# luzbetak/rag-faiss-embedding

Measured on NVIDIA B200. Metric: queries/sec @k=10 (flat L2, 384-d), higher is better.
Workload: dtype bf16 tensor-core candidates + f32 exact re-rank

## Files before the change

### rag-faiss-embedding_b200/csrc/gemm_topk_sm100.cu

```cuda
#include <cuda.h>
#include <math.h>
#include <stdlib.h>

#include "common.cuh"
#include "rerank.cuh"

namespace b2f {

namespace k2 {

constexpr int BM = 128;
constexpr int BN = 256;
constexpr int BK = 64;
constexpr int UMMA_K = 16;
constexpr int STAGES_HEAP = 3;
constexpr int STAGES_LIST = 4;
constexpr int STAGES_QRES = 3;
constexpr int QRES_MAX_KB = 6;
constexpr int LIST_CAP_MIN = 128;
constexpr int JSLOTS = 16;
constexpr int A_BYTES = BM * BK * 2;
constexpr int B_BYTES = BN * BK * 2;
constexpr int STAGE_BYTES = A_BYTES + B_BYTES;
constexpr int EPI_THREADS = 128;
// ... 759 lines not shown
#pragma unroll
                    for (int c4 = 0; c4 < 8; c4++)
                        *reinterpret_cast<uint4*>(st + ((c4 ^ (lane & 7)) << 2)) = make_uint4(r[4 * c4], r[4 * c4 + 1], r[4 * c4 + 2], r[4 * c4 + 3]);
                    uint32_t m = mask;
                    while (m) {
                        const int j = __ffs(m) - 1;
                        m &= m - 1;
                        const float sdot = __uint_as_float(st[((((j >> 2) ^ (lane & 7)) << 2)) + (j & 3)]);
                        const float key = L2 ? fmaf(-2.f, sdot, tbc[j]) : tbc[j] - sdot;
                        if (cnt < la.cap) mylist[cnt] = make_uint2(__float_as_uint(key), (uint32_t)(rowc + j));
                        cnt++;
                        if (jv == 1) {
                            best[JSLOTS - 1] = fminf(best[JSLOTS - 1], key);
                        } else if (key < best[JSLOTS - 1]) {
                            float nb[JSLOTS];
#pragma unroll
                            for (int i = 0; i < JSLOTS; i++) nb[i] = fmaxf(i > 0 ? best[i - 1] : -kInf, fminf(best[i], key));
#pragma unroll
                            for (int i = 0; i < JSLOTS; i++) best[i] = nb[i];
                        }
                    }
                }
            };
            const int seg_tiles = seg_tiles_of(sgi);
#pragma unroll 1
            for (int t = 0; t < seg_tiles; t++, gt++) {
                const int acc = gt & 1;
                const uint32_t acc_phase = (gt >> 1) & 1;
                if (la.early && active && t >= 2 && (t < 8 || (t < 32 && (t & 3) == 0) || (t & la.period_mask) == 0)) refresh(true);
                const uint32_t rmask = t == 0 ? 0xffffffffu : (t == 1 ? 0x55555555u
                                     : ((!la.early && (t < 8 || (t < 32 && (t & 3) == 0) || (t & 15) == 0)) ? 1u : 0u));
                mbar_wait(&bias_full[acc], acc_phase);
                mbar_wait(&tmem_full[acc], acc_phase);
                tc_fence_after();
                const int32_t row0 = tile_row0[acc] + half * COLS;
                const float* tb = bias + acc * BN + half * COLS;
                const uint32_t tile_taddr = lane_taddr + (uint32_t)(acc * BN + half * COLS);
                uint32_t ra[32], rb[32];
                tmem_ld32(tile_taddr, ra);
#pragma unroll 1
                for (int c = 0; c < COLS / 32; c += 2) {
                    tmem_ld_wait();
                    tmem_ld32(tile_taddr + (uint32_t)((c + 1) * 32), rb);
                    process(ra, ((rmask >> c) & 1u) != 0u, false, tb + c * 32, row0 + c * 32);
                    tmem_ld_wait();
                    if (c + 2 < COLS / 32) tmem_ld32(tile_taddr + (uint32_t)((c + 2) * 32), ra);
                    process(rb, ((rmask >> (c + 1)) & 1u) != 0u, t == 0 && c == 0, tb + (c + 1) * 32, row0 + (c + 1) * 32);
                }
                tc_fence_before();
                __syncwarp();
                if (lane == 0) {
                    if constexpr (PAIR) {
                        mbar_arrive(&bias_empty[acc]);
                        mbar_arrive_cluster(&tmem_empty[acc], 0);
                    } else {
                        mbar_arrive(&tmem_empty[acc]);
                    }
                }
            }
            if (warp == 4 && lane == 0) K2_STAMP(4);
            if (active) {
                const int have = cnt <= la.cap ? cnt : 0;
                refresh(true);
                int w = 0;
#pragma unroll 1
                for (int i0 = 0; i0 < have; i0 += 16) {
                    uint2 e[16];
#pragma unroll
                    for (int u = 0; u < 16; u++) e[u] = (i0 + u < have) ? mylist[i0 + u] : make_uint2(0x7f800000u, 0u);
#pragma unroll
                    for (int u = 0; u < 16; u++)
                        if (i0 + u < have && __uint_as_float(e[u].x) <= thr) mylist[w++] = e[u];
                }
                la.counts[(int64_t)qrow * la.nl_stride + vsplit] = cnt > la.cap ? cnt : w;
                la.final_thr[(int64_t)qrow * la.nl_stride + vsplit] = thr;
            }
            if (warp == 4 && lane == 0) K2_STAMP(5);
            }
        } else {
            const int qrow = seg[0].qtile * BM + tid;
            const bool active = qrow < nq;
            for (int j = 0; j < KP; j++) {
                heap_k[j * EPI_THREADS + tid] = FLT_MAX;
                heap_i[j * EPI_THREADS + tid] = -1;
            }
            float thr = FLT_MAX;
            const int heap_tiles = seg_tiles_of(0);
            for (int t = 0; t < heap_tiles; t++) {
                const int acc = t & 1;
                const uint32_t acc_phase = (t >> 1) & 1;
                mbar_wait(&bias_full[acc], acc_phase);
                mbar_wait(&tmem_full[acc], acc_phase);
                tc_fence_after();
                const int32_t row0 = tile_row0[acc];
                const float* tb = bias + acc * BN;
                const uint32_t tile_taddr = lane_taddr + (uint32_t)(acc * BN);
#pragma unroll 1
                for (int c = 0; c < BN / 32; c++) {
                    uint32_t r[32];
                    tmem_ld32(tile_taddr + (uint32_t)(c * 32), r);
                    tmem_ld_wait();
                    const float* tbc = tb + c * 32;
                    const uint32_t mask = active ? chunk_mask(r, tbc, thr) : 0u;
                    uint32_t um = __reduce_or_sync(kFull, mask);
                    while (um) {
                        const int j = __ffs(um) - 1;
                        um &= um - 1;
                        const uint32_t v = pick(r, j);
                        if (mask & (1u << j)) {
                            const float sdot = __uint_as_float(v);
                            const float key = L2 ? fmaf(-2.f, sdot, tbc[j]) : tbc[j] - sdot;
                            if (key < thr) thr = heap_push<KP>(heap_k, heap_i, tid, key, row0 + c * 32 + j);
                        }
                    }
                }
                tc_fence_before();
                __syncwarp();
                if (lane == 0) mbar_arrive(&tmem_empty[acc]);
            }
            if (active) {
                for (int m = KP - 1; m > 0; m--) {
                    const float lk_ = heap_k[m * EPI_THREADS + tid];
                    const int32_t li_ = heap_i[m * EPI_THREADS + tid];
                    heap_k[m * EPI_THREADS + tid] = heap_k[tid];
                    heap_i[m * EPI_THREADS + tid] = heap_i[tid];
                    heap_sift_down_n<KP>(heap_k, heap_i, tid, m, lk_, li_);
                }
                float* ok = pk + ((int64_t)qrow * nsplits + split) * KP;
                int32_t* oi = pi + ((int64_t)qrow * nsplits + split) * KP;
                for (int j = 0; j < KP; j++) {
                    ok[j] = heap_k[j * EPI_THREADS + tid];
                    oi[j] = heap_i[j * EPI_THREADS + tid];
                }
            }
        }
    }
    tc_fence_before();
    __syncthreads();
    if constexpr (PAIR) cluster_sync_all();
    if (threadIdx.x == 0) K2_STAMP(6);
    if (warp == 2) {
        tc_fence_after();
        if constexpr (PAIR)
            asm volatile("tcgen05.dealloc.cta_group::2.sync.aligned.b32 %0, %1;" ::"r"(tmem_base), "r"((uint32_t)TMEM_COLS) : "memory");
        else
            asm volatile("tcgen05.dealloc.cta_group::1.sync.aligned.b32 %0, %1;" ::"r"(tmem_base), "r"((uint32_t)TMEM_COLS) : "memory");
        if (lane == 0) K2_STAMP(7);
    }
}

constexpr int MERGE_THREADS = kRerankThreads;
constexpr int MERGE_MAX = 4096;
constexpr int RANK_MAX = 1024;
constexpr int KP_MAX = 256;
static_assert(MERGE_MAX == kRangeHitsMax, "range search stages as many entries per query as the merge holds");

__device__ __forceinline__ int block_count_le(const unsigned long long* comp, int M, unsigned long long bound, int* s_cnt,
                                              int it, int tid, int lane) {
    if (tid == 0) s_cnt[(it + 1) % 3] = 0;
    int c = 0;
    for (int i = tid; i < M; i += MERGE_THREADS) c += comp[i] <= bound ? 1 : 0;
    c = __reduce_add_sync(kFull, c);
    if (lane == 0 && c) atomicAdd(&s_cnt[it % 3], c);
    __syncthreads();
    return s_cnt[it % 3];
}

__device__ __forceinline__ void radix_pick(int* s_hist, int* s_wsum, int* s_sel, int shift, unsigned int& lo, int& need,
                                           int tid, int lane, int warp) {
    __syncthreads();
    const int h = s_hist[tid];
    int incl = h;
#pragma unroll
    for (int d = 1; d < 32; d <<= 1) {
        const int up = __shfl_up_sync(kFull, incl, d);
        if (lane >= d) incl += up;
    }
    if (lane == 31) s_wsum[warp] = incl;
    __syncthreads();
    int base = 0;
    for (int w = 0; w < warp; w++) base += s_wsum[w];
    incl += base;
    if (incl >= need && incl - h < need) {
        s_sel[0] = tid;
        s_sel[1] = need - (incl - h);
    }
    __syncthreads();
    lo |= (unsigned int)s_sel[0] << shift;
    need = s_sel[1];
    __syncthreads();
}

__global__ void __launch_bounds__(MERGE_THREADS)
merge_lists_kernel(const uint2* __restrict__ cand, const int32_t* __restrict__ counts, const float* __restrict__ final_thr,
                   int nl_stride, int tile_queries, int ntile_units, int total_units, int halves, int kp, int list_cap,
                   int cap_entries, unsigned long long* __restrict__ total_entries, const uint8_t* __restrict__ only_flagged,
                   const RerankArgs ra) {
    extern __shared__ __align__(16) unsigned long long comp[];
    if (only_flagged && !only_flagged[blockIdx.x]) return;
    __shared__ int s_off[2 * kNumSMs + 2];
    __shared__ int s_cnt[3];
    __shared__ int s_nsurv, s_nrest;
    __shared__ int s_hist[MERGE_THREADS], s_wsum[MERGE_THREADS / 32], s_sel[2];
    __shared__ int s_ovf;
    __shared__ unsigned int s_tc_enc;
    const int cap_c = cap_entries > RANK_MAX ? cap_entries : RANK_MAX;
    unsigned long long* surv = comp + cap_c;
    float* sk = reinterpret_cast<float*>(surv + KP_MAX);
    int32_t* si = reinterpret_cast<int32_t*>(sk + RANK_MAX);
    unsigned short* owner = reinterpret_cast<unsigned short*>(si + RANK_MAX);
    float* ek = reinterpret_cast<float*>(comp);
    int32_t* ei = reinterpret_cast<int32_t*>(ek + RANK_MAX);
    const int q = blockIdx.x, tid = threadIdx.x, lane = tid & 31, warp = tid >> 5;
    const int tile = q / tile_queries;
    int nsplits;
    {
        const TileInfo ti = tile_info(tile, ntile_units, total_units, 0, halves);
        nsplits = (ti.nfw + ti.nsw) * halves;
    }
    if (tid == 0) {
        s_tc_enc = 0xffffffffu;
        s_ovf = 0;
        s_nsurv = 0;
        s_nrest = 0;
        s_cnt[0] = 0;
    }
    __syncthreads();
    {
        float tc = 3.0e38f;
        int o = 0;
        for (int s2 = tid; s2 < nsplits; s2 += MERGE_THREADS) {
            int c = counts[(int64_t)q * nl_stride + s2];
            tc = fminf(tc, final_thr[(int64_t)q * nl_stride + s2]);
            if (c > list_cap) {
                c = list_cap;
                o = 1;
            }
            s_off[s2 + 1] = c;
        }
#pragma unroll
        for (int d = 16; d >= 1; d >>= 1) tc = fminf(tc, __shfl_xor_sync(kFull, tc, d));
        o = __reduce_or_sync(kFull, o);
        if (lane == 0) {
            atomicMin(&s_tc_enc, enc_key(tc));
            if (o) s_ovf = 1;
        }
    }
    __syncthreads();
    if (warp == 0) {
        int run = 0;
        for (int s0 = 0; s0 < nsplits; s0 += 32) {
            const int s2 = s0 + lane;
            const int c = s2 < nsplits ? s_off[s2 + 1] : 0;
            int incl = c;
#pragma unroll
            for (int d = 1; d < 32; d <<= 1) {
                const int up = __shfl_up_sync(kFull, incl, d);
                if (lane >= d) incl += up;
            }
            __syncwarp();
            if (s2 < nsplits) s_off[s2 + 1] = run + incl;
            run += __shfl_sync(kFull, incl, 31);
        }
        if (lane == 0) {
            s_off[0] = 0;
            if (total_entries) atomicAdd(total_entries, (unsigned long long)run);
            if (run > cap_entries && (ra.range || !ra.certify)) s_ovf = 1;
        }
    }
    __syncthreads();
    if (ra.out_map && ra.out_map[q] < 0) return;
    if (s_ovf) {
        if (tid == 0) rerank_record_failure(ra, q, true);
        return;
    }
    int M = s_off[nsplits];
    const bool big = M > cap_entries;
    if (big) {
        unsigned int lo = 0;
        int need = kp;
#pragma unroll 1
        for (int pass = 0; pass < 4; pass++) {
            const int shift = 24 - 8 * pass;
            s_hist[tid] = 0;
            __syncthreads();
#pragma unroll 1
            for (int l = 0; l < nsplits; l++) {
                const int c = s_off[l + 1] - s_off[l];
                const uint2* p = cand + ((int64_t)q * nl_stride + l) * list_cap;
                for (int j0 = 0; j0 < c; j0 += MERGE_THREADS) {
                    const int j = j0 + tid;
                    const unsigned int key = j < c ? enc_key(__uint_as_float(p[j].x)) : 0u;
                    const bool in = j < c && (pass == 0 || (key >> (shift + 8)) == (lo >> (shift + 8)));
                    const unsigned int bin = (key >> shift) & 255u;
                    const unsigned int peers = __match_any_sync(kFull, in ? bin : 256u + (unsigned)lane);
                    if (in && lane == __ffs(peers) - 1) atomicAdd(&s_hist[bin], __popc(peers));
                }
            }
            radix_pick(s_hist, s_wsum, s_sel, shift, lo, need, tid, lane, warp);
        }
#pragma unroll 1
        for (int l = 0; l < nsplits; l++) {
            const int c = s_off[l + 1] - s_off[l];
            const uint2* p = cand + ((int64_t)q * nl_stride + l) * list_cap;
            for (int j = tid; j < c; j += MERGE_THREADS) {
                const uint2 e = p[j];
                const unsigned int key = enc_key(__uint_as_float(e.x));
                if (key <= lo) {
                    const int slot = atomicAdd(&s_nrest, 1);
                    if (slot < cap_entries) comp[slot] = ((unsigned long long)key << 32) | (unsigned long long)e.y;
                }
            }
        }
        __syncthreads();
        M = s_nrest;
        __syncthreads();
        if (tid == 0) s_nrest = 0;
        if (M > cap_entries) {
            if (tid == 0) rerank_record_failure(ra, q, true);
            return;
        }
        __syncthreads();
    } else {
    for (int l = tid; l < nsplits; l += MERGE_THREADS) {
        const int o = s_off[l], e = s_off[l + 1];
        for (int i = o; i < e; i++) owner[i] = (unsigned short)l;
    }
    __syncthreads();
    for (int i0 = tid; i0 < M; i0 += 4 * MERGE_THREADS) {
        uint2 e[4];
#pragma unroll
        for (int u = 0; u < 4; u++) {
            const int i = i0 + u * MERGE_THREADS;
            e[u] = make_uint2(0u, 0u);
            if (i < M) {
                const int l = owner[i];
                e[u] = cand[((int64_t)q * nl_stride + l) * list_cap + (i - s_off[l])];
            }
        }
#pragma unroll
        for (int u = 0; u < 4; u++) {
            const int i = i0 + u * MERGE_THREADS;
            if (i < M) comp[i] = ((unsigned long long)enc_key(__uint_as_float(e[u].x)) << 32) | (unsigned long long)e[u].y;
        }
    }
    }
    __syncthreads();
    if (M <= MERGE_THREADS) {
        if (tid < M) {
            const unsigned long long mine = comp[tid];
            int rank = 0;
            for (int j = 0; j < M; j++) rank += comp[j] < mine ? 1 : 0;
            sk[rank] = dec_key((uint32_t)(mine >> 32));
            si[rank] = (int32_t)(uint32_t)(mine & 0xffffffffu);
        }
    } else {
        unsigned long long T = ~0ull;
        int it = 0;
        unsigned int lo = 0;
        int need = kp;
#pragma unroll 1
        for (int pass = 0; pass < 4; pass++) {
            const int shift = 24 - 8 * pass;
            s_hist[tid] = 0;
            __syncthreads();
            for (int i0 = 0; i0 < M; i0 += MERGE_THREADS) {
                const int i = i0 + tid;
                const unsigned int key = i < M ? (unsigned int)(comp[i] >> 32) : 0u;
                const bool in = i < M && (pass == 0 || (key >> (shift + 8)) == (lo >> (shift + 8)));
                const unsigned int bin = (key >> shift) & 255u;
                const unsigned int peers = __match_any_sync(kFull, in ? bin : 256u + (unsigned)lane);
                if (in && lane == __ffs(peers) - 1) atomicAdd(&s_hist[bin], __popc(peers));
            }
            radix_pick(s_hist, s_wsum, s_sel, shift, lo, need, tid, lane, warp);
        }
        const unsigned long long kbits = (unsigned long long)lo << 32;
        T = kbits | 0xffffffffull;
        if (block_count_le(comp, M, T, s_cnt, it++, tid, lane) > kp) {
            unsigned int ilo = 0, ihi = 0xffffffffu;
            while (ilo < ihi) {
                const unsigned int mid = ilo + ((ihi - ilo) >> 1);
                const int total = block_count_le(comp, M, kbits | mid, s_cnt, it++, tid, lane);
                if (total >= kp) ihi = mid;
                else ilo = mid + 1;
            }
            T = kbits | ilo;
        }
        for (int i = tid; i < M; i += MERGE_THREADS) {
            const unsigned long long v = comp[i];
            if (v <= T) {
                const int slot = atomicAdd(&s_nsurv, 1);
                if (slot < kp) surv[slot] = v;
            } else if (M <= RANK_MAX) {
                const int slot = kp + atomicAdd(&s_nrest, 1);
                if (slot < RANK_MAX) {
                    sk[slot] = dec_key((uint32_t)(v >> 32));
                    si[slot] = (int32_t)(uint32_t)(v & 0xffffffffu);
                }
            }
        }
        __syncthreads();
        const int ns = s_nsurv < kp ? s_nsurv : kp;
        for (int t = tid; t < ns; t += MERGE_THREADS) {
            const unsigned long long mine = surv[t];
            int rank = 0;
            for (int j = 0; j < ns; j++) rank += surv[j] < mine ? 1 : 0;
            sk[rank] = dec_key((uint32_t)(mine >> 32));
            si[rank] = (int32_t)(uint32_t)(mine & 0xffffffffu);
        }
    }
    __syncthreads();
    const float tc = dec_key(s_tc_enc);
    const int nc1 = M < kp ? M : kp;
    const float bound1 = (M > kp || big) ? fminf(sk[kp - 1], tc) : tc;
    __shared__ float s_tau_last;
    bool cert = false;
    if (ra.range) {
        if (M <= RANK_MAX) cert = rerank_block(ra, q, sk, si, M, tc, false, ek, ei, &s_tau_last);
        else if (tid == 0) s_tau_last = FLT_MAX;
    } else {
        if (ra.certify && ra.stage1 >= ra.k && ra.stage1 < nc1)
            cert = rerank_block(ra, q, sk, si, ra.stage1, fminf(sk[ra.stage1], tc), false, ek, ei, &s_tau_last);
        if (!cert) cert = rerank_block(ra, q, sk, si, nc1, bound1, M < kp, ek, ei, &s_tau_last);
        if (!cert && ra.certify && !big && M > kp && M <= RANK_MAX) {
            cert = rerank_block(ra, q, sk, si, M, tc, false, ek, ei, &s_tau_last);
            if (tid == 0 && cert) atomicAdd(ra.fail_count + 4, 1);
        }
    }
    if (tid == 0 && ra.certify && !cert) rerank_record_failure(ra, q, false, s_tau_last);
}

constexpr int WM_WARPS = 8;
constexpr int WM_MAX = 128;
constexpr int WM_LISTS = 64;

__device__ __forceinline__ bool warp_rerank(const RerankArgs& a, int q, const float* sk, const int32_t* si, int nc, float bound,
                                            bool all_rows, float* ek, int32_t* ei, int lane, float& tau_out) {
    const float* qv = a.q + (int64_t)q * a.d;
    const bool l2 = a.metric == B2F_METRIC_L2;
    const int sl = lane & 7;
    for (int c0 = 0; c0 < nc; c0 += 4) {
        const int c = c0 + (lane >> 3);
        int32_t id = c < nc ? si[c] : -1;
        if ((int64_t)id >= a.ntotal) id = -1;
        const float key = exact_key_8lanes(a, qv, id, sl, l2);
        if (sl == 0 && c < nc) {
            const bool ok = id >= 0 && !(key != key);
            ek[c] = ok ? key : FLT_MAX;
            ei[c] = ok ? id : -1;
        }
    }
    __syncwarp();
    float tau = FLT_MAX;
    for (int t = lane; t < nc; t += 32) {
        const float mk = ek[t];
        const int32_t mi = ei[t];
        int rank = 0;
        for (int j = 0; j < nc; j++) {
            const float ok_ = ek[j];
            const int32_t oi_ = ei[j];
            rank += (cand_less(ok_, oi_, mk, mi) || (ok_ == mk && oi_ == mi && j < t)) ? 1 : 0;
        }
        if (rank < a.k) {
            const int64_t o = (int64_t)q * a.k + rank;
            a.D[o] = mi < 0 ? (l2 ? FLT_MAX : -FLT_MAX) : (l2 ? mk : -mk);
            a.I[o] = mi < 0 ? -1 : (int64_t)mi + a.id_offset;
        }
        if (rank == a.k - 1) tau = mk;
    }
    for (int t = nc + lane; t < a.k; t += 32) {
        a.D[(int64_t)q * a.k + t] = l2 ? FLT_MAX : -FLT_MAX;
        a.I[(int64_t)q * a.k + t] = -1;
    }
#pragma unroll
    for (int d = 16; d >= 1; d >>= 1) tau = fminf(tau, __shfl_xor_sync(kFull, tau, d));
    __syncwarp();
    tau_out = tau;
    return all_rows || rerank_certified(a, q, tau, bound);
}

__global__ void __launch_bounds__(WM_WARPS * 32)
merge_lists_warp_kernel(const uint2* __restrict__ cand, const int32_t* __restrict__ counts, const float* __restrict__ final_thr,
                        int nl_stride, int tile_queries, int ntile_units, int total_units, int halves, int kp, int list_cap,
                        unsigned long long* __restrict__ total_entries, uint8_t* __restrict__ big_flag, int nq, const RerankArgs ra) {
    __shared__ __align__(16) unsigned long long s_comp[WM_WARPS][WM_MAX];
    __shared__ float s_sk[WM_WARPS][WM_MAX], s_ek[WM_WARPS][WM_MAX];
    __shared__ int32_t s_si[WM_WARPS][WM_MAX], s_ei[WM_WARPS][WM_MAX];
    const int warp = threadIdx.x >> 5, lane = threadIdx.x & 31;
    const int q = blockIdx.x * WM_WARPS + warp;
    if (q >= nq) return;
    unsigned long long* comp = s_comp[warp];
    float* sk = s_sk[warp];
    int32_t* si = s_si[warp];
    int nlists;
    {
        const TileInfo ti = tile_info(q / tile_queries, ntile_units, total_units, 0, halves);
        nlists = (ti.nfw + ti.nsw) * halves;
    }
    int c0 = 0, c1 = 0;
    float tc = 3.0e38f;
    bool ovf = false;
    if (lane < nlists) {
        c0 = counts[(int64_t)q * nl_stride + lane];
        tc = fminf(tc, final_thr[(int64_t)q * nl_stride + lane]);
    }
    if (lane + 32 < nlists) {
        c1 = counts[(int64_t)q * nl_stride + lane + 32];
        tc = fminf(tc, final_thr[(int64_t)q * nl_stride + lane + 32]);
    }
    ovf = c0 > list_cap || c1 > list_cap;
    int i0 = c0, i1 = c1;
#pragma unroll
    for (int d = 1; d < 32; d <<= 1) {
        const int u0 = __shfl_up_sync(kFull, i0, d), u1 = __shfl_up_sync(kFull, i1, d);
        if (lane >= d) { i0 += u0; i1 += u1; }
    }
    const int tot0 = __shfl_sync(kFull, i0, 31), M = tot0 + __shfl_sync(kFull, i1, 31);
#pragma unroll
    for (int d = 16; d >= 1; d >>= 1) tc = fminf(tc, __shfl_xor_sync(kFull, tc, d));
    ovf = __any_sync(kFull, ovf);
    if (lane == 0 && total_entries) atomicAdd(total_entries, (unsigned long long)(ovf ? 0 : M));
    if (ovf || M > WM_MAX) {
        if (lane == 0) big_flag[q] = 1;
        return;
    }
    if (lane == 0) big_flag[q] = 0;
    {
        const uint2* l0 = cand + ((int64_t)q * nl_stride + lane) * list_cap;
        const int o0 = i0 - c0;
        for (int i = 0; i < c0; i++) {
            const uint2 e = l0[i];
            comp[o0 + i] = ((unsigned long long)enc_key(__uint_as_float(e.x)) << 32) | (unsigned long long)e.y;
        }
        const uint2* l1 = cand + ((int64_t)q * nl_stride + lane + 32) * list_cap;
        const int o1 = tot0 + i1 - c1;
        for (int i = 0; i < c1; i++) {
            const uint2 e = l1[i];
            comp[o1 + i] = ((unsigned long long)enc_key(__uint_as_float(e.x)) << 32) | (unsigned long long)e.y;
        }
    }
    __syncwarp();
    for (int t = lane; t < M; t += 32) {
        const unsigned long long mine = comp[t];
        int rank = 0;
        for (int j = 0; j < M; j++) rank += comp[j] < mine ? 1 : 0;
        sk[rank] = dec_key((uint32_t)(mine >> 32));
        si[rank] = (int32_t)(uint32_t)(mine & 0xffffffffu);
    }
    __syncwarp();
    const int nc1 = M < kp ? M : kp;
    const float bound1 = (M > kp) ? fminf(sk[kp - 1], tc) : tc;
    bool cert = false;
    float tau = FLT_MAX;
    if (ra.certify && ra.stage1 >= ra.k && ra.stage1 < nc1)
        cert = warp_rerank(ra, q, sk, si, ra.stage1, fminf(sk[ra.stage1], tc), false, s_ek[warp], s_ei[warp], lane, tau);
    if (!cert) cert = warp_rerank(ra, q, sk, si, nc1, bound1, M < kp, s_ek[warp], s_ei[warp], lane, tau);
    if (!cert && ra.certify && M > kp) {
        cert = warp_rerank(ra, q, sk, si, M, tc, false, s_ek[warp], s_ei[warp], lane, tau);
        if (lane == 0 && cert) atomicAdd(ra.fail_count + 4, 1);
    }
    if (lane == 0 && ra.certify && !cert) rerank_record_failure(ra, q, false, tau);
}

typedef CUresult (*EncodeTiledFn)(CUtensorMap*, CUtensorMapDataType, cuuint32_t, void*, const cuuint64_t*, const cuuint64_t*,
                                  const cuuint32_t*, const cuuint32_t*, CUtensorMapInterleave, CUtensorMapSwizzle,
                                  CUtensorMapL2promotion, CUtensorMapFloatOOBfill);

static EncodeTiledFn get_encode() {
    static EncodeTiledFn fn = nullptr;
    if (!fn) {
        void* p = nullptr;
        cudaDriverEntryPointQueryResult qres;
        if (cudaGetDriverEntryPoint("cuTensorMapEncodeTiled", &p, cudaEnableDefault, &qres) == cudaSuccess &&
            qres == cudaDriverEntryPointSuccess)
            fn = reinterpret_cast<EncodeTiledFn>(p);
    }
    return fn;
}
// ... 244 lines not shown
    plan->units = units;
    plan->nsplits = units / plan->tile_units;
    if (!plan->list_mode) {
        plan->nlists = plan->nsplits;
        plan->list_j = kp;
        plan->list_g = 1;
        plan->list_cap = 0;
        return B2F_OK;
    }
    plan->nlists = nseg_max * halves;
    const int j = nv_min;
    plan->list_j = j;
    plan->list_g = (kp + j - 1) / j;
    {
        int r = 2 * ((units + plan->tile_units - 1) / plan->tile_units);
        if (r < 2) r = 2;
        if (r > 512) r = 512;
        const char* e = getenv("B200FLAT_ROUND_TILES");
        if (e && atoi(e) >= 1 && atoi(e) <= 4096) r = atoi(e);
        plan->round_tiles = r;
    }
    {
        const double rows_per_list = (double)n * plan->tile_units / units / halves;
        const double expected = 32.0 + (j + 2.5) * log(rows_per_list > 64.0 ? rows_per_list / 32.0 : 2.0);
        int cap = (int)(2.5 * expected);
        cap = (cap + 63) / 64 * 64;
        if (cap < k2::LIST_CAP_MIN) cap = k2::LIST_CAP_MIN;
        if (cap > 1024) cap = 1024;
        plan->list_cap = cap;
    }
    return B2F_OK;
}

int plan_unit_work(int T, int U, int R, int64_t ntiles, int kp, int unit, int32_t* seg_info, int64_t* tiles, int64_t cap, int32_t* counts) {
    if (T < 1 || U < T || R < 1 || ntiles < 0 || kp < 1 || unit < 0 || unit >= U || !seg_info || !counts) return -1;
    k2::Seg seg[2];
    const int nseg = k2::unit_segments(unit, T, U, kp, k2::EPI_WARPS_LIST / 4, seg);
    for (int s = 0; s < nseg; s++) {
        seg_info[7 * s + 0] = seg[s].qtile;
        seg_info[7 * s + 1] = seg[s].slot;
        seg_info[7 * s + 2] = seg[s].nv;
        seg_info[7 * s + 3] = (int32_t)seg[s].p0;
        seg_info[7 * s + 4] = (int32_t)seg[s].p1;
        seg_info[7 * s + 5] = seg[s].j;
        seg_info[7 * s + 6] = seg[s].g;
        k2::SegIter it;
        it.init(seg[s].p0, seg[s].p1, U, R, ntiles);
        int32_t c = 0;
        for (int64_t t; (t = it.next()) >= 0; c++)
            if (tiles && c < cap) tiles[(int64_t)s * cap + c] = t;
        counts[s] = c;
    }
    return nseg;
}

int launch_tensor_scan(const __nv_bfloat16* scan, int64_t dpad, const float* norms, int64_t n, int metric,
                       const __nv_bfloat16* qb, int nq, int nq_pad, const TensorScanPlan& plan, float* pk, int32_t* pi,
                       const TensorScanLists& lists, cudaStream_t st) {
    struct MapKey {
        const void* base;
        uint64_t inner, rows;
        uint32_t box;
        bool operator==(const MapKey& o) const { return base == o.base && inner == o.inner && rows == o.rows && box == o.box; }
    };
    static thread_local MapKey kq{}, kx{};
    static thread_local CUtensorMap mq, mx;
    const MapKey nkq{qb, (uint64_t)dpad, (uint64_t)nq_pad, (uint32_t)k2::BM};
    const MapKey nkx{scan, (uint64_t)dpad, (uint64_t)n, (uint32_t)(plan.pair_mode ? k2::BN / 2 : k2::BN)};
    if (!(nkq == kq)) {
        B2F_TRY(k2::make_map(&mq, qb, (uint64_t)dpad, (uint64_t)nq_pad, (uint64_t)dpad, k2::BM));
        kq = nkq;
    }
    if (!(nkx == kx)) {
        B2F_TRY(k2::make_map(&mx, scan, (uint64_t)dpad, (uint64_t)n, (uint64_t)dpad, nkx.box));
        kx = nkx;
    }
    const int kblocks = (int)(dpad / k2::BK);
    const bool l2 = metric == B2F_METRIC_L2;
    k2::ListArgs la{};
    if (plan.list_mode) {
        la.shared_thr = lists.shared_thr;
        la.cand = reinterpret_cast<uint2*>(lists.cand);
        la.counts = lists.counts;
        la.kp = plan.kp;
        la.nl_stride = plan.nlists;
        la.cap = plan.list_cap;
        la.final_thr = lists.final_thr;
        {
            static int early = -1;
            if (early < 0) {
                const char* e = getenv("B200FLAT_EARLY_REFRESH");
                early = (e && e[0] == '0') ? 0 : 1;
            }
            la.early = early;
            static int period = -1;
            if (period < 0) {
                const char* e = getenv("B200FLAT_REFRESH_PERIOD");
                period = e ? atoi(e) : 32;
                if (period != 2 && period != 4 && period != 8 && period != 16 && period != 32 && period != 64 && period != 128) period = 32;
            }
            la.period_mask = period - 1;
            static int keep = -1;
            if (keep < 0) {
                const char* e = getenv("B200FLAT_L2_KEEP");
                keep = (e && e[0] == '1') ? 1 : 0;
            }
            la.l2_keep = keep;
            static int die_mode = -1;
            if (die_mode < 0) {
                const char* e = getenv("B200FLAT_DIE_MODE");
                die_mode = e ? atoi(e) : 1;
                if (die_mode < 0 || die_mode > 3) die_mode = 1;
            }
            la.die_mode = (lists.die_ctr && plan.tile_units > 1) ? die_mode : 0;
            la.die_ctr = lists.die_ctr;
            la.bal_T = plan.tile_units;
            la.bal_U = plan.units;
            la.bal_R = plan.round_tiles;
            la.range_thr = lists.range_thr;
        }
        if (plan.pair_mode)
            return l2 ? k2::launch_k2<0, true, true, true, true>(mq, mx, norms, n, nq, kblocks, plan, pk, pi, la, st)
                      : k2::launch_k2<0, false, true, true, true>(mq, mx, norms, n, nq, kblocks, plan, pk, pi, la, st);
        if (kblocks <= k2::QRES_MAX_KB)
            return l2 ? k2::launch_k2<0, true, true, true>(mq, mx, norms, n, nq, kblocks, plan, pk, pi, la, st)
                      : k2::launch_k2<0, false, true, true>(mq, mx, norms, n, nq, kblocks, plan, pk, pi, la, st);
        return l2 ? k2::launch_k2<0, true, true, false>(mq, mx, norms, n, nq, kblocks, plan, pk, pi, la, st)
                  : k2::launch_k2<0, false, true, false>(mq, mx, norms, n, nq, kblocks, plan, pk, pi, la, st);
    }
    if (plan.kp == 32)
        return l2 ? k2::launch_k2<32, true, false, false>(mq, mx, norms, n, nq, kblocks, plan, pk, pi, la, st)
                  : k2::launch_k2<32, false, false, false>(mq, mx, norms, n, nq, kblocks, plan, pk, pi, la, st);
    if (plan.kp == 64)
        return l2 ? k2::launch_k2<64, true, false, false>(mq, mx, norms, n, nq, kblocks, plan, pk, pi, la, st)
                  : k2::launch_k2<64, false, false, false>(mq, mx, norms, n, nq, kblocks, plan, pk, pi, la, st);
    set_error("tensor scan: k' = %d not supported", plan.kp);
    return B2F_EINVAL;
}

int launch_merge_lists(const TensorScanLists& lists, int nq, const TensorScanPlan& plan, unsigned long long* total_entries,
                       const RerankArgs& ra, cudaStream_t st) {
    if (nq <= 0) return B2F_OK;
    if (plan.kp > k2::KP_MAX || plan.nlists > 2 * kNumSMs) {
        set_error("merge: k' = %d / %d lists per query not supported", plan.kp, plan.nlists);
        return B2F_EINVAL;
    }
    int cap_entries = plan.nlists * plan.list_cap;
    const int expect = 4 * (plan.kp + 3 * plan.nlists);
    if (cap_entries > expect) cap_entries = expect;
    if (cap_entries < k2::RANK_MAX) cap_entries = k2::RANK_MAX;
    if (cap_entries > k2::MERGE_MAX) cap_entries = k2::MERGE_MAX;
    const int cap_c = cap_entries > k2::RANK_MAX ? cap_entries : k2::RANK_MAX;
    const size_t smem = (size_t)cap_c * 8 + (size_t)k2::KP_MAX * 8 + (size_t)k2::RANK_MAX * 8 + (size_t)cap_entries * 2;
    {
        static bool configured[kMaxDevices] = {};
        const int dev = current_device_slot();
        std::lock_guard<std::mutex> lk(launch_cache_mutex());
        if (!configured[dev]) {
            B2F_CUDA(cudaFuncSetAttribute(k2::merge_lists_kernel, cudaFuncAttributeMaxDynamicSharedMemorySize,
                                          (int)((size_t)k2::MERGE_MAX * 10 + (size_t)k2::KP_MAX * 8 + (size_t)k2::RANK_MAX * 8)));
            configured[dev] = true;
        }
    }
    const uint8_t* only_flagged = nullptr;
    static int warp_env = -1;
    if (warp_env < 0) {
        const char* e = getenv("B200FLAT_WARP_MERGE");
        warp_env = e ? atoi(e) : 8192;
    }
    if (warp_env > 0 && nq >= warp_env && lists.big_flag && plan.nlists <= k2::WM_LISTS && plan.kp <= k2::WM_MAX / 2 && ra.D &&
        !ra.range && !ra.out_map) {
        k2::merge_lists_warp_kernel<<<(nq + k2::WM_WARPS - 1) / k2::WM_WARPS, k2::WM_WARPS * 32, 0, st>>>(
            reinterpret_cast<const uint2*>(lists.cand), lists.counts, lists.final_thr, plan.nlists, plan.pair_mode ? 2 * k2::BM : k2::BM,
            plan.tile_units, plan.units, k2::EPI_WARPS_LIST / 4, plan.kp, plan.list_cap, total_entries, lists.big_flag, nq, ra);
        B2F_CUDA(cudaGetLastError());
        only_flagged = lists.big_flag;
        total_entries = nullptr;
    }
    k2::merge_lists_kernel<<<nq, k2::MERGE_THREADS, smem, st>>>(reinterpret_cast<const uint2*>(lists.cand), lists.counts, lists.final_thr,
                                                               plan.nlists, plan.pair_mode ? 2 * k2::BM : k2::BM, plan.tile_units, plan.units,
                                                               k2::EPI_WARPS_LIST / 4, plan.kp, plan.list_cap, cap_entries, total_entries,
                                                               only_flagged, ra);
    B2F_CUDA(cudaGetLastError());
    return B2F_OK;
}

int launch_range_collect(const TensorScanLists& lists, int nq, const TensorScanPlan& plan, float tau, const RerankArgs& ra,
                         float* skey, int32_t* sid, int32_t* staged, int32_t* count, int32_t* scan_list, int32_t* scan_n,
                         cudaStream_t st) {
    if (nq <= 0) return B2F_OK;
    if (!plan.list_mode || plan.nlists > 2 * kNumSMs) {
        set_error("range collect: a LIST-mode plan of at most %d lists per query is required", 2 * kNumSMs);
        return B2F_EINVAL;
    }
    k2::range_collect_kernel<<<nq, k2::MERGE_THREADS, 0, st>>>(reinterpret_cast<const uint2*>(lists.cand), lists.counts, lists.range_thr,
                                                               plan.nlists, plan.pair_mode ? 2 * k2::BM : k2::BM, plan.tile_units,
                                                               plan.units, k2::EPI_WARPS_LIST / 4, plan.list_cap, tau, ra, skey, sid,
                                                               staged, count, scan_list, scan_n);
    B2F_CUDA(cudaGetLastError());
    return B2F_OK;
}

}

#ifdef B2F_K2_TRACE
extern "C" __attribute__((visibility("default"))) int b2f_debug_k2_trace(unsigned long long* out, int n) {
    if (n > 2 * b2f::kNumSMs * 12) n = 2 * b2f::kNumSMs * 12;
    if (cudaMemcpyFromSymbol(out, b2f::k2::g_k2_trace, (size_t)n * 8) != cudaSuccess) return -1;
    static unsigned long long zeros[2 * b2f::kNumSMs * 12] = {};
    return cudaMemcpyToSymbol(b2f::k2::g_k2_trace, zeros, sizeof(zeros)) == cudaSuccess ? 0 : -1;
}
#endif
```

### rag-faiss-embedding_b200/csrc/rerank.cuh

```cuda
#pragma once
#include "common.cuh"

namespace b2f {

constexpr int kRerankThreads = 256;

__device__ __forceinline__ float exact_key_8lanes(const RerankArgs& a, const float* __restrict__ qv, int32_t id, int sl, bool l2) {
    float acc = 0.f;
    if (id >= 0) {
        if (a.rows_f32 && (a.d & 3) == 0) {
            const float* x = a.rows_f32 + (int64_t)id * a.d;
            for (int j0 = sl * 4; j0 < a.d; j0 += 128) {
                float4 xv[4], qq[4];
#pragma unroll
                for (int u = 0; u < 4; u++) {
                    const int j = j0 + 32 * u;
                    xv[u] = j < a.d ? __ldg(reinterpret_cast<const float4*>(x + j)) : make_float4(0.f, 0.f, 0.f, 0.f);
                }
#pragma unroll
                for (int u = 0; u < 4; u++) {
                    const int j = j0 + 32 * u;
                    qq[u] = j < a.d ? __ldg(reinterpret_cast<const float4*>(qv + j)) : make_float4(0.f, 0.f, 0.f, 0.f);
                }
#pragma unroll
                for (int u = 0; u < 4; u++) {
                    if (l2) {
                        const float t0 = xv[u].x - qq[u].x, t1 = xv[u].y - qq[u].y, t2 = xv[u].z - qq[u].z, t3 = xv[u].w - qq[u].w;
                        acc = fmaf(t0, t0, acc); acc = fmaf(t1, t1, acc); acc = fmaf(t2, t2, acc); acc = fmaf(t3, t3, acc);
                    } else {
                        acc = fmaf(xv[u].x, qq[u].x, acc); acc = fmaf(xv[u].y, qq[u].y, acc);
                        acc = fmaf(xv[u].z, qq[u].z, acc); acc = fmaf(xv[u].w, qq[u].w, acc);
                    }
                }
            }
        } else if (!a.rows_f32 && (a.d & 7) == 0) {
            const __nv_bfloat16* x = a.rows_bf16 + (int64_t)id * a.pitch_bf16;
            for (int j0 = sl * 8; j0 < a.d; j0 += 128) {
                uint4 w[2];
#pragma unroll
                for (int u = 0; u < 2; u++) {
                    const int j = j0 + 64 * u;
                    w[u] = j < a.d ? __ldg(reinterpret_cast<const uint4*>(x + j)) : make_uint4(0u, 0u, 0u, 0u);
                }
#pragma unroll
                for (int u = 0; u < 2; u++) {
                    const int j = j0 + 64 * u;
                    if (j < a.d) {
                        const uint32_t ww[4] = {w[u].x, w[u].y, w[u].z, w[u].w};
                        const float4 qa = __ldg(reinterpret_cast<const float4*>(qv + j));
                        const float4 qb = __ldg(reinterpret_cast<const float4*>(qv + j + 4));
                        const float qq[8] = {qa.x, qa.y, qa.z, qa.w, qb.x, qb.y, qb.z, qb.w};
                        float mm[8] = {0.f, 0.f, 0.f, 0.f, 0.f, 0.f, 0.f, 0.f};
                        if (a.centre) {
                            const float4 ma = __ldg(reinterpret_cast<const float4*>(a.centre + j));
                            const float4 mb = __ldg(reinterpret_cast<const float4*>(a.centre + j + 4));
                            mm[0] = ma.x; mm[1] = ma.y; mm[2] = ma.z; mm[3] = ma.w; mm[4] = mb.x; mm[5] = mb.y; mm[6] = mb.z; mm[7] = mb.w;
                        }
#pragma unroll
                        for (int h = 0; h < 4; h++) {
                            const float x0 = mm[2 * h] + __uint_as_float(ww[h] << 16), x1 = mm[2 * h + 1] + __uint_as_float(ww[h] & 0xffff0000u);
                            if (l2) {
                                const float t0 = x0 - qq[2 * h], t1 = x1 - qq[2 * h + 1];
                                acc = fmaf(t0, t0, acc); acc = fmaf(t1, t1, acc);
                            } else {
                                acc = fmaf(x0, qq[2 * h], acc); acc = fmaf(x1, qq[2 * h + 1], acc);
                            }
                        }
                    }
                }
            }
        } else {
            for (int j = sl; j < a.d; j += 8) {
                const float xv = a.rows_f32 ? a.rows_f32[(int64_t)id * a.d + j]
                                            : (a.centre ? a.centre[j] : 0.f) + __bfloat162float(a.rows_bf16[(int64_t)id * a.pitch_bf16 + j]);
                if (l2) {
                    const float t = xv - qv[j];
                    acc = fmaf(t, t, acc);
                } else {
                    acc = fmaf(xv, qv[j], acc);
                }
            }
        }
    }
    acc += __shfl_xor_sync(kFull, acc, 4);
    acc += __shfl_xor_sync(kFull, acc, 2);
    acc += __shfl_xor_sync(kFull, acc, 1);
    return l2 ? acc : -acc;
}

__device__ __forceinline__ bool rerank_certified(const RerankArgs& a, int q, float tau, float bound) {
    const bool l2 = a.metric == B2F_METRIC_L2;
    const float qn2 = a.qnorm[q];
    const float qn = sqrtf(qn2);
    const float eq = a.qerr[q];
    const float gam = 4.f * (float)(a.d + 16) * 5.9604645e-8f;
    if (l2) {
        const float nu = gam * (2.f * qn * a.max_row_norm + qn2 + a.max_row_norm * a.max_row_norm);
        const float c = bound + qn2 - nu;
        const float L = sqrtf(fmaxf(c, 0.f)) - eq - a.max_row_err;
        return L > 0.f && L * L * (1.f - 4e-7f) > tau;
    }
    const float cq = a.qconst ? a.qconst[q] : 0.f;
    const float xmax = a.max_row_norm + a.max_row_err + a.mu_norm;
    const float nu = gam * qn * a.max_row_norm + 2.4e-7f * (a.mu_norm * (xmax + qn + eq + a.mu_norm) + qn * a.max_row_norm);
    const float U = -bound + cq + nu + (qn + eq) * a.max_row_err + a.max_row_norm * eq;
    return U < -tau;
}

__device__ __forceinline__ bool rerank_block(const RerankArgs& a, int q, const float* ck, const int32_t* ci, int nc, float bound,
                                             bool all_rows, float* ek, int32_t* ei, float* tau_out = nullptr) {
    __shared__ float s_tau;
    __shared__ int s_cert;
    const int lane = threadIdx.x & 31;
    const float* qv = a.q + (int64_t)q * a.d;
    const bool l2 = a.metric == B2F_METRIC_L2;
    const int64_t orow = a.out_map ? (int64_t)a.out_map[q] : (int64_t)q;
    if (threadIdx.x == 0) s_tau = FLT_MAX;
    __syncthreads();
    const int sl = lane & 7;
    for (int c0 = 0; c0 < nc; c0 += kRerankThreads / 8) {
        const int c = c0 + (threadIdx.x >> 3);
        int32_t id = c < nc ? ci[c] : -1;
        if ((int64_t)id >= a.ntotal) id = -1;
        const float key = exact_key_8lanes(a, qv, id, sl, l2);
        if (sl == 0 && c < nc) {
            const bool ok = id >= 0 && !(key != key);
            ek[c] = ok ? key : FLT_MAX;
            ei[c] = ok ? id : -1;
        }
    }
    __syncthreads();
    for (int t = threadIdx.x; t < nc; t += kRerankThreads) {
        const float mk = ek[t];
        const int32_t mi = ei[t];
        int rank = 0;
        for (int j = 0; j < nc; j++) {
            const float ok_ = ek[j];
            const int32_t oi_ = ei[j];
            rank += (cand_less(ok_, oi_, mk, mi) || (ok_ == mk && oi_ == mi && j < t)) ? 1 : 0;
        }
        if (rank < a.k) {
            if (a.D) {
                const int64_t o = orow * a.k + rank;
                a.D[o] = mi < 0 ? (l2 ? FLT_MAX : -FLT_MAX) : (l2 ? mk : -mk);
                a.I[o] = mi < 0 ? -1 : (int64_t)mi + a.id_offset;
            } else {
                a.out_key[(int64_t)q * a.k + rank] = mk;
                a.out_id[(int64_t)q * a.k + rank] = mi;
            }
        }
        if (rank == a.k - 1) s_tau = mk;
    }
    for (int t = nc + threadIdx.x; t < a.k; t += kRerankThreads) {
        if (a.D) {
            a.D[orow * a.k + t] = l2 ? FLT_MAX : -FLT_MAX;
            a.I[orow * a.k + t] = -1;
        } else {
            a.out_key[(int64_t)q * a.k + t] = FLT_MAX;
            a.out_id[(int64_t)q * a.k + t] = -1;
        }
    }
    __syncthreads();
    if (threadIdx.x == 0) {
        const bool certified = all_rows || rerank_certified(a, q, s_tau, bound);
        s_cert = certified ? 1 : 0;
        if (tau_out) *tau_out = s_tau;
    }
    __syncthreads();
    return s_cert != 0;
}

__device__ __forceinline__ void rerank_record_failure(const RerankArgs& a, int q, bool overflowed, float tau = FLT_MAX) {
    const int slot = atomicAdd(a.fail_count, 1);
    a.fail_list[slot] = a.out_map ? a.out_map[q] : q + a.q_base;
    if (a.fail_tau) a.fail_tau[slot] = tau;
    if (overflowed) atomicAdd(a.fail_count + 1, 1);
}

}
```

Baseline: 1.594 million.

## Template merge kernel on block size and pick 128 or 256 threads by occupancy

```diff
diff --git a/rag-faiss-embedding_b200/csrc/gemm_topk_sm100.cu b/rag-faiss-embedding_b200/csrc/gemm_topk_sm100.cu
--- a/rag-faiss-embedding_b200/csrc/gemm_topk_sm100.cu
+++ b/rag-faiss-embedding_b200/csrc/gemm_topk_sm100.cu
@@ -935,25 +935,34 @@
 constexpr int MERGE_THREADS = kRerankThreads;
 constexpr int MERGE_MAX = 4096;
 constexpr int RANK_MAX = 1024;
+constexpr int RANK_DIRECT = 256;
 constexpr int KP_MAX = 256;
 static_assert(MERGE_MAX == kRangeHitsMax, "range search stages as many entries per query as the merge holds");
 
+template <int T>
 __device__ __forceinline__ int block_count_le(const unsigned long long* comp, int M, unsigned long long bound, int* s_cnt,
                                               int it, int tid, int lane) {
     if (tid == 0) s_cnt[(it + 1) % 3] = 0;
     int c = 0;
-    for (int i = tid; i < M; i += MERGE_THREADS) c += comp[i] <= bound ? 1 : 0;
+    for (int i = tid; i < M; i += T) c += comp[i] <= bound ? 1 : 0;
     c = __reduce_add_sync(kFull, c);
     if (lane == 0 && c) atomicAdd(&s_cnt[it % 3], c);
     __syncthreads();
     return s_cnt[it % 3];
 }
 
+template <int T>
 __device__ __forceinline__ void radix_pick(int* s_hist, int* s_wsum, int* s_sel, int shift, unsigned int& lo, int& need,
                                            int tid, int lane, int warp) {
+    constexpr int B = 256 / T;
     __syncthreads();
-    const int h = s_hist[tid];
-    int incl = h;
+    int h[B], own = 0;
+#pragma unroll
+    for (int b = 0; b < B; b++) {
+        h[b] = s_hist[tid * B + b];
+        own += h[b];
+    }
+    int incl = own;
 #pragma unroll
     for (int d = 1; d < 32; d <<= 1) {
         const int up = __shfl_up_sync(kFull, incl, d);
@@ -961,12 +970,15 @@
     }
     if (lane == 31) s_wsum[warp] = incl;
     __syncthreads();
-    int base = 0;
-    for (int w = 0; w < warp; w++) base += s_wsum[w];
-    incl += base;
-    if (incl >= need && incl - h < need) {
-        s_sel[0] = tid;
-        s_sel[1] = need - (incl - h);
+    int start = incl - own;
+    for (int w = 0; w < warp; w++) start += s_wsum[w];
+#pragma unroll
+    for (int b = 0; b < B; b++) {
+        if (start < need && start + h[b] >= need) {
+            s_sel[0] = tid * B + b;
+            s_sel[1] = need - start;
+        }
+        start += h[b];
     }
     __syncthreads();
     lo |= (unsigned int)s_sel[0] << shift;
@@ -974,17 +986,19 @@
     __syncthreads();
 }
 
-__global__ void __launch_bounds__(MERGE_THREADS)
+template <int T>
+__global__ void __launch_bounds__(T, T == 128 ? 9 : 4)
 merge_lists_kernel(const uint2* __restrict__ cand, const int32_t* __restrict__ counts, const float* __restrict__ final_thr,
                    int nl_stride, int tile_queries, int ntile_units, int total_units, int halves, int kp, int list_cap,
                    int cap_entries, unsigned long long* __restrict__ total_entries, const uint8_t* __restrict__ only_flagged,
                    const RerankArgs ra) {
+    static_assert(T == 128 || T == 256, "the radix select's 256 bins are spread over the block");
     extern __shared__ __align__(16) unsigned long long comp[];
     if (only_flagged && !only_flagged[blockIdx.x]) return;
     __shared__ int s_off[2 * kNumSMs + 2];
     __shared__ int s_cnt[3];
     __shared__ int s_nsurv, s_nrest;
-    __shared__ int s_hist[MERGE_THREADS], s_wsum[MERGE_THREADS / 32], s_sel[2];
+    __shared__ int s_hist[256], s_wsum[T / 32], s_sel[2];
     __shared__ int s_ovf;
     __shared__ unsigned int s_tc_enc;
     const int cap_c = cap_entries > RANK_MAX ? cap_entries : RANK_MAX;
@@ -1012,7 +1026,7 @@
     {
         float tc = 3.0e38f;
         int o = 0;
-        for (int s2 = tid; s2 < nsplits; s2 += MERGE_THREADS) {
+        for (int s2 = tid; s2 < nsplits; s2 += T) {
             int c = counts[(int64_t)q * nl_stride + s2];
             tc = fminf(tc, final_thr[(int64_t)q * nl_stride + s2]);
             if (c > list_cap) {
@@ -1065,13 +1079,13 @@
 #pragma unroll 1
         for (int pass = 0; pass < 4; pass++) {
             const int shift = 24 - 8 * pass;
-            s_hist[tid] = 0;
+            for (int b = tid; b < 256; b += T) s_hist[b] = 0;
             __syncthreads();
 #pragma unroll 1
             for (int l = 0; l < nsplits; l++) {
                 const int c = s_off[l + 1] - s_off[l];
                 const uint2* p = cand + ((int64_t)q * nl_stride + l) * list_cap;
-                for (int j0 = 0; j0 < c; j0 += MERGE_THREADS) {
+                for (int j0 = 0; j0 < c; j0 += T) {
                     const int j = j0 + tid;
                     const unsigned int key = j < c ? enc_key(__uint_as_float(p[j].x)) : 0u;
                     const bool in = j < c && (pass == 0 || (key >> (shift + 8)) == (lo >> (shift + 8)));
@@ -1080,13 +1094,13 @@
                     if (in && lane == __ffs(peers) - 1) atomicAdd(&s_hist[bin], __popc(peers));
                 }
             }
-            radix_pick(s_hist, s_wsum, s_sel, shift, lo, need, tid, lane, warp);
+            radix_pick<T>(s_hist, s_wsum, s_sel, shift, lo, need, tid, lane, warp);
         }
 #pragma unroll 1
         for (int l = 0; l < nsplits; l++) {
             const int c = s_off[l + 1] - s_off[l];
             const uint2* p = cand + ((int64_t)q * nl_stride + l) * list_cap;
-            for (int j = tid; j < c; j += MERGE_THREADS) {
+            for (int j = tid; j < c; j += T) {
                 const uint2 e = p[j];
                 const unsigned int key = enc_key(__uint_as_float(e.x));
                 if (key <= lo) {
@@ -1105,16 +1119,16 @@
         }
         __syncthreads();
     } else {
-    for (int l = tid; l < nsplits; l += MERGE_THREADS) {
+    for (int l = tid; l < nsplits; l += T) {
         const int o = s_off[l], e = s_off[l + 1];
         for (int i = o; i < e; i++) owner[i] = (unsigned short)l;
     }
     __syncthreads();
-    for (int i0 = tid; i0 < M; i0 += 4 * MERGE_THREADS) {
+    for (int i0 = tid; i0 < M; i0 += 4 * T) {
         uint2 e[4];
 #pragma unroll
         for (int u = 0; u < 4; u++) {
-            const int i = i0 + u * MERGE_THREADS;
+            const int i = i0 + u * T;
             e[u] = make_uint2(0u, 0u);
             if (i < M) {
                 const int l = owner[i];
@@ -1123,31 +1137,31 @@
         }
 #pragma unroll
         for (int u = 0; u < 4; u++) {
-            const int i = i0 + u * MERGE_THREADS;
+            const int i = i0 + u * T;
             if (i < M) comp[i] = ((unsigned long long)enc_key(__uint_as_float(e[u].x)) << 32) | (unsigned long long)e[u].y;
         }
     }
     }
     __syncthreads();
-    if (M <= MERGE_THREADS) {
-        if (tid < M) {
-            const unsigned long long mine = comp[tid];
+    if (M <= RANK_DIRECT) {
+        for (int t = tid; t < M; t += T) {
+            const unsigned long long mine = comp[t];
             int rank = 0;
             for (int j = 0; j < M; j++) rank += comp[j] < mine ? 1 : 0;
             sk[rank] = dec_key((uint32_t)(mine >> 32));
             si[rank] = (int32_t)(uint32_t)(mine & 0xffffffffu);
         }
     } else {
-        unsigned long long T = ~0ull;
+        unsigned long long Tb = ~0ull;
         int it = 0;
         unsigned int lo = 0;
         int need = kp;
 #pragma unroll 1
         for (int pass = 0; pass < 4; pass++) {
             const int shift = 24 - 8 * pass;
-            s_hist[tid] = 0;
+            for (int b = tid; b < 256; b += T) s_hist[b] = 0;
             __syncthreads();
-            for (int i0 = 0; i0 < M; i0 += MERGE_THREADS) {
+            for (int i0 = 0; i0 < M; i0 += T) {
                 const int i = i0 + tid;
                 const unsigned int key = i < M ? (unsigned int)(comp[i] >> 32) : 0u;
                 const bool in = i < M && (pass == 0 || (key >> (shift + 8)) == (lo >> (shift + 8)));
@@ -1155,23 +1169,23 @@
                 const unsigned int peers = __match_any_sync(kFull, in ? bin : 256u + (unsigned)lane);
                 if (in && lane == __ffs(peers) - 1) atomicAdd(&s_hist[bin], __popc(peers));
             }
-            radix_pick(s_hist, s_wsum, s_sel, shift, lo, need, tid, lane, warp);
+            radix_pick<T>(s_hist, s_wsum, s_sel, shift, lo, need, tid, lane, warp);
         }
         const unsigned long long kbits = (unsigned long long)lo << 32;
-        T = kbits | 0xffffffffull;
-        if (block_count_le(comp, M, T, s_cnt, it++, tid, lane) > kp) {
+        Tb = kbits | 0xffffffffull;
+        if (block_count_le<T>(comp, M, Tb, s_cnt, it++, tid, lane) > kp) {
             unsigned int ilo = 0, ihi = 0xffffffffu;
             while (ilo < ihi) {
                 const unsigned int mid = ilo + ((ihi - ilo) >> 1);
-                const int total = block_count_le(comp, M, kbits | mid, s_cnt, it++, tid, lane);
+                const int total = block_count_le<T>(comp, M, kbits | mid, s_cnt, it++, tid, lane);
                 if (total >= kp) ihi = mid;
                 else ilo = mid + 1;
             }
-            T = kbits | ilo;
-        }
-        for (int i = tid; i < M; i += MERGE_THREADS) {
+            Tb = kbits | ilo;
+        }
+        for (int i = tid; i < M; i += T) {
             const unsigned long long v = comp[i];
-            if (v <= T) {
+            if (v <= Tb) {
                 const int slot = atomicAdd(&s_nsurv, 1);
                 if (slot < kp) surv[slot] = v;
             } else if (M <= RANK_MAX) {
@@ -1184,7 +1198,7 @@
         }
         __syncthreads();
         const int ns = s_nsurv < kp ? s_nsurv : kp;
-        for (int t = tid; t < ns; t += MERGE_THREADS) {
+        for (int t = tid; t < ns; t += T) {
             const unsigned long long mine = surv[t];
             int rank = 0;
             for (int j = 0; j < ns; j++) rank += surv[j] < mine ? 1 : 0;
@@ -1199,14 +1213,14 @@
     __shared__ float s_tau_last;
     bool cert = false;
     if (ra.range) {
-        if (M <= RANK_MAX) cert = rerank_block(ra, q, sk, si, M, tc, false, ek, ei, &s_tau_last);
+        if (M <= RANK_MAX) cert = rerank_block<T>(ra, q, sk, si, M, tc, false, ek, ei, &s_tau_last);
         else if (tid == 0) s_tau_last = FLT_MAX;
     } else {
         if (ra.certify && ra.stage1 >= ra.k && ra.stage1 < nc1)
-            cert = rerank_block(ra, q, sk, si, ra.stage1, fminf(sk[ra.stage1], tc), false, ek, ei, &s_tau_last);
-        if (!cert) cert = rerank_block(ra, q, sk, si, nc1, bound1, M < kp, ek, ei, &s_tau_last);
+            cert = rerank_block<T>(ra, q, sk, si, ra.stage1, fminf(sk[ra.stage1], tc), false, ek, ei, &s_tau_last);
+        if (!cert) cert = rerank_block<T>(ra, q, sk, si, nc1, bound1, M < kp, ek, ei, &s_tau_last);
         if (!cert && ra.certify && !big && M > kp && M <= RANK_MAX) {
-            cert = rerank_block(ra, q, sk, si, M, tc, false, ek, ei, &s_tau_last);
+            cert = rerank_block<T>(ra, q, sk, si, M, tc, false, ek, ei, &s_tau_last);
             if (tid == 0 && cert) atomicAdd(ra.fail_count + 4, 1);
         }
     }
@@ -1757,14 +1771,49 @@
     if (cap_entries > k2::MERGE_MAX) cap_entries = k2::MERGE_MAX;
     const int cap_c = cap_entries > k2::RANK_MAX ? cap_entries : k2::RANK_MAX;
     const size_t smem = (size_t)cap_c * 8 + (size_t)k2::KP_MAX * 8 + (size_t)k2::RANK_MAX * 8 + (size_t)cap_entries * 2;
+    static int force_threads = -1;
+    if (force_threads < 0) {
+        const char* e = getenv("B200FLAT_MERGE_THREADS");
+        force_threads = e ? atoi(e) : 0;
+        if (force_threads != 128 && force_threads != 256) force_threads = 0;
+    }
+    int threads = 256;
     {
-        static bool configured[kMaxDevices] = {};
+        struct Occ {
+            size_t smem;
+            int b128, b256;
+        };
+        constexpr int kOccSlots = 8;
+        static Occ occ[kMaxDevices][kOccSlots] = {};
+        static int nsm[kMaxDevices] = {};
         const int dev = current_device_slot();
         std::lock_guard<std::mutex> lk(launch_cache_mutex());
-        if (!configured[dev]) {
-            B2F_CUDA(cudaFuncSetAttribute(k2::merge_lists_kernel, cudaFuncAttributeMaxDynamicSharedMemorySize,
-                                          (int)((size_t)k2::MERGE_MAX * 10 + (size_t)k2::KP_MAX * 8 + (size_t)k2::RANK_MAX * 8)));
-            configured[dev] = true;
+        if (!nsm[dev]) {
+            const int max_smem = (int)((size_t)k2::MERGE_MAX * 10 + (size_t)k2::KP_MAX * 8 + (size_t)k2::RANK_MAX * 8);
+            B2F_CUDA(cudaFuncSetAttribute(k2::merge_lists_kernel<128>, cudaFuncAttributeMaxDynamicSharedMemorySize, max_smem));
+            B2F_CUDA(cudaFuncSetAttribute(k2::merge_lists_kernel<256>, cudaFuncAttributeMaxDynamicSharedMemorySize, max_smem));
+            int d = 0, n = 0;
+            B2F_CUDA(cudaGetDevice(&d));
+            B2F_CUDA(cudaDeviceGetAttribute(&n, cudaDevAttrMultiProcessorCount, d));
+            nsm[dev] = n;
+        }
+        Occ* o = nullptr;
+        for (int i = 0; i < kOccSlots && !o; i++)
+            if (occ[dev][i].smem == smem) o = &occ[dev][i];
+        if (!o) {
+            int slot = 0;
+            while (slot < kOccSlots - 1 && occ[dev][slot].smem) slot++;
+            o = &occ[dev][slot];
+            B2F_CUDA(cudaOccupancyMaxActiveBlocksPerMultiprocessor(&o->b128, k2::merge_lists_kernel<128>, 128, smem));
+            B2F_CUDA(cudaOccupancyMaxActiveBlocksPerMultiprocessor(&o->b256, k2::merge_lists_kernel<256>, 256, smem));
+            o->smem = smem;
+        }
+        if (force_threads) {
+            threads = force_threads;
+        } else if (o->b128 > 0) {
+            const int64_t w128 = ((int64_t)nq + (int64_t)o->b128 * nsm[dev] - 1) / ((int64_t)o->b128 * nsm[dev]);
+            const int64_t w256 = o->b256 > 0 ? ((int64_t)nq + (int64_t)o->b256 * nsm[dev] - 1) / ((int64_t)o->b256 * nsm[dev]) : INT64_MAX;
+            if (w128 < w256) threads = 128;
         }
     }
     const uint8_t* only_flagged = nullptr;
@@ -1782,10 +1831,10 @@
         only_flagged = lists.big_flag;
         total_entries = nullptr;
     }
-    k2::merge_lists_kernel<<<nq, k2::MERGE_THREADS, smem, st>>>(reinterpret_cast<const uint2*>(lists.cand), lists.counts, lists.final_thr,
-                                                               plan.nlists, plan.pair_mode ? 2 * k2::BM : k2::BM, plan.tile_units, plan.units,
-                                                               k2::EPI_WARPS_LIST / 4, plan.kp, plan.list_cap, cap_entries, total_entries,
-                                                               only_flagged, ra);
+    auto kern = threads == 128 ? k2::merge_lists_kernel<128> : k2::merge_lists_kernel<256>;
+    kern<<<nq, threads, smem, st>>>(reinterpret_cast<const uint2*>(lists.cand), lists.counts, lists.final_thr, plan.nlists,
+                                    plan.pair_mode ? 2 * k2::BM : k2::BM, plan.tile_units, plan.units, k2::EPI_WARPS_LIST / 4,
+                                    plan.kp, plan.list_cap, cap_entries, total_entries, only_flagged, ra);
     B2F_CUDA(cudaGetLastError());
     return B2F_OK;
 }
diff --git a/rag-faiss-embedding_b200/csrc/rerank.cuh b/rag-faiss-embedding_b200/csrc/rerank.cuh
--- a/rag-faiss-embedding_b200/csrc/rerank.cuh
+++ b/rag-faiss-embedding_b200/csrc/rerank.cuh
@@ -107,6 +107,7 @@
     return U < -tau;
 }
 
+template <int T = kRerankThreads>
 __device__ __forceinline__ bool rerank_block(const RerankArgs& a, int q, const float* ck, const int32_t* ci, int nc, float bound,
                                              bool all_rows, float* ek, int32_t* ei, float* tau_out = nullptr) {
     __shared__ float s_tau;
@@ -118,7 +119,7 @@
     if (threadIdx.x == 0) s_tau = FLT_MAX;
     __syncthreads();
     const int sl = lane & 7;
-    for (int c0 = 0; c0 < nc; c0 += kRerankThreads / 8) {
+    for (int c0 = 0; c0 < nc; c0 += T / 8) {
         const int c = c0 + (threadIdx.x >> 3);
         int32_t id = c < nc ? ci[c] : -1;
         if ((int64_t)id >= a.ntotal) id = -1;
@@ -130,7 +131,7 @@
         }
     }
     __syncthreads();
-    for (int t = threadIdx.x; t < nc; t += kRerankThreads) {
+    for (int t = threadIdx.x; t < nc; t += T) {
         const float mk = ek[t];
         const int32_t mi = ei[t];
         int rank = 0;
@@ -151,7 +152,7 @@
         }
         if (rank == a.k - 1) s_tau = mk;
     }
-    for (int t = nc + threadIdx.x; t < a.k; t += kRerankThreads) {
+    for (int t = nc + threadIdx.x; t < a.k; t += T) {
         if (a.D) {
             a.D[orow * a.k + t] = l2 ? FLT_MAX : -FLT_MAX;
             a.I[orow * a.k + t] = -1;
```

New measurement: 1.600 million (median of 6 runs). Within noise of the previous version (+0.3%).
